# NVIDIA/nvidia-resiliency-ext

Hardware: AMD Instinct MI355X
Metric: generate_report_latency_us (lower is better)
Workload: dtype f32; 1 GPU; 8 ranks x 64 sections x 10000 samples per report, ring capacity 10000, relative+individual scores, gather_on_rank0; logical_ranks_per_gpu=8, rows_per_gpu=512, exchange=none (single process)

## Files before the change

nvidia-resiliency-ext_amd/csrc/nvrx_straggler.hip:

```cpp
#include <hip/hip_runtime.h>
#include <hip/hip_ext.h>

#include <algorithm>
#include <atomic>
#include <chrono>
#include <thread>
#include <cmath>
#include <cstdarg>
#include <cstdio>
#include <cstdlib>
#include <cstring>
#include <deque>
#include <mutex>
#include <string>
#include <unordered_map>
#include <utility>
#include <vector>

#include "nvrx_straggler.h"

namespace {

thread_local std::string g_err;

// ... 282 lines not shown
    mn = min(mn, dpp<DPP_QUAD_2301>(0xFFFFFFFFu, mn));
    mx = max(mx, dpp0<DPP_QUAD_2301>(mx));
    mn = min(mn, dpp<DPP_ROW_SHR4>(0xFFFFFFFFu, mn));
    mx = max(mx, dpp0<DPP_ROW_SHR4>(mx));
    mn = min(mn, dpp<DPP_ROW_SHR8>(0xFFFFFFFFu, mn));
    mx = max(mx, dpp0<DPP_ROW_SHR8>(mx));
    mn = min(mn, dpp<DPP_BCAST15>(0xFFFFFFFFu, mn));
    mx = max(mx, dpp0<DPP_BCAST15>(mx));
    mn = min(mn, dpp<DPP_BCAST31>(0xFFFFFFFFu, mn));
    mx = max(mx, dpp0<DPP_BCAST31>(mx));
    mn = (uint32_t)__builtin_amdgcn_readlane((int)mn, 63);
    mx = (uint32_t)__builtin_amdgcn_readlane((int)mx, 63);
}

__device__ __forceinline__ double recip_count(uint32_t c) {
    const double d = (double)c;
    double r = __builtin_amdgcn_rcp(d);
    r = fma(fma(-d, r, 1.0), r, r);
    r = fma(fma(-d, r, 1.0), r, r);
    return c ? r : __builtin_inf();
}

template <int THREADS, int VPT>
__global__ __launch_bounds__(THREADS) void k_row_stats(const float *__restrict__ samples,
                                                       const uint32_t *__restrict__ counts,
                                                       const uint8_t *__restrict__ kinds, int row_stride,
                                                       float *__restrict__ stats, Epilogue ep, int uniform_n) {
    constexpr int WAVES = THREADS / 64;
    constexpr int HIST_BITS = THREADS >= 512 ? NVRX_HIST_BITS_WIDE : 11;
    constexpr int HIST_BINS = 1 << HIST_BITS;
    constexpr int PER = HIST_BINS / THREADS;
    constexpr int G = THREADS / 64;
    constexpr int NKEY = VPT * 4;
    constexpr int CAND_MAX = 256;
    constexpr int CAND_ONE = 64;
    static_assert(HIST_BINS % THREADS == 0, "THREADS must divide the histogram size");
    static_assert(THREADS >= CAND_MAX, "candidate list is initialised one word per thread");

    __shared__ __attribute__((aligned(16))) uint32_t s_hist[HIST_BINS];
    __shared__ __attribute__((aligned(16))) uint32_t s_sum[THREADS];
    __shared__ __attribute__((aligned(16))) uint32_t s_cand[CAND_MAX];
    __shared__ __attribute__((aligned(16))) uint32_t s_lt[CAND_MAX];
    __shared__ __attribute__((aligned(16))) double s_d[2 * WAVES];
    __shared__ __attribute__((aligned(16))) uint32_t s_mm[4];
    __shared__ uint32_t s_cur[1];

    const int row = ep.rows_active ? (int)(blockIdx.x / ep.rows_active) * ep.rows_per_rank + (int)(blockIdx.x % ep.rows_active)
                                   : (int)blockIdx.x;
    const int tid = threadIdx.x;
    const int lane = tid & 63;
// ... 487 lines not shown
                                              r_min, r_max, r_med, r_avg, r_std, (float)n, weight, (float)path};
#pragma unroll
            for (int q = 0; q < ROW_GRANULES; q++)
                __hip_atomic_store(g8 + q, tag | (unsigned long long)__float_as_uint(vals[q]), __ATOMIC_RELAXED,
                                   __HIP_MEMORY_SCOPE_AGENT);
        } else if (ep.send) {
            const int lr = row / ep.rows_per_rank;
            float *s = ep.send + (size_t)lr * ep.L;
            const int g = row_gid;
            if (g >= 0 && g < ep.KS) {
                s[g] = n ? r_med : -1.0f;
                s[ep.KS + g] = n ? h : __builtin_nanf("");
                if (g < ep.K) s[2 * ep.KS + g] = weight;
            }
            if (row - lr * ep.rows_per_rank == 0) s[ep.L - 1] = ep.names_ok;
        }
    }
    NVRX_PHASE(8);
#ifdef NVRX_PHASE_CLOCKS
    if (threadIdx.x == 0 && blockIdx.x < 4096) g_phase[blockIdx.x][9] = wall_clock64();
#endif
}

struct StagedSample {
    uint32_t row_slot;
    float value;
};

__global__ void k_scatter(const uint32_t *__restrict__ h_counts, const StagedSample *__restrict__ h_entries,
                          int n_entries, float *__restrict__ samples, int row_stride,
                          uint32_t *__restrict__ d_counts, int rows, const uint8_t *__restrict__ h_kinds,
                          uint8_t *__restrict__ d_kinds, const int32_t *__restrict__ h_gid,
                          int32_t *__restrict__ d_gid, uint32_t *__restrict__ done_cnt, uint32_t *done_word,
                          uint32_t ticket) {
    const int i = blockIdx.x * blockDim.x + threadIdx.x;
    if (i < n_entries) {
        const StagedSample e = h_entries[i];
        samples[(size_t)(e.row_slot >> 16) * (size_t)row_stride + (e.row_slot & 0xFFFFu)] = e.value;
    }
    if (i < rows) {
        d_counts[i] = h_counts[i];
        if (h_kinds) {
            d_kinds[i] = h_kinds[i];
            d_gid[i] = h_gid[i];
        }
    }
// ... 350 lines not shown
    float *send;
    nvrx_f4 *stats_out;
    uint32_t *err;
    int n_blocks, rows_active, rows_per_rank, local_ranks;
    float names_ok;
    uint32_t epoch;
    unsigned long long timeout_ticks;
    int poll_naps;
};

__device__ __forceinline__ float wait_granule(const unsigned long long *p, const GatherArgs &g, unsigned long long t0) {
    uint32_t spins = 0;
    for (;;) {
        const unsigned long long x = __hip_atomic_load(p, __ATOMIC_RELAXED, __HIP_MEMORY_SCOPE_AGENT);
        if ((uint32_t)(x >> 32) == g.epoch) return __uint_as_float((uint32_t)x);
        __builtin_amdgcn_s_sleep(2);
        if ((++spins & 0xFFu) == 0u && wall_clock64() - t0 > g.timeout_ticks) {
            __hip_atomic_store(g.err, g.epoch, __ATOMIC_RELAXED, __HIP_MEMORY_SCOPE_SYSTEM);
            return __builtin_nanf("");
        }
    }
}

template <int NTHR>
__global__ __launch_bounds__(NTHR) void k_score1(ScoreArgs a, int fence, PeerArgs pa, GatherArgs ga) {
    extern __shared__ __attribute__((aligned(16))) unsigned char s_raw[];

    const int K = a.K, S = a.S, KS = K + S, R = a.R;
    const int L = NVRX_TABLE_LEN(K, S);
    const int W = NVRX_SCORE_LEN(S);
    const int nout = R * W;
    const int nout4 = (nout + 3) & ~3;
    float *s_min = reinterpret_cast<float *>(s_raw);
    float *s_out = s_min + ((KS + 3) & ~3);
    uint8_t *s_fl = reinterpret_cast<uint8_t *>(s_out + nout4);
    float *s_tab = a.tab_in_lds ? reinterpret_cast<float *>(s_fl + ((nout + 15) & ~15)) : nullptr;
    float *s_send = a.tab_in_lds ? s_tab + ((R * L + 3) & ~3) : nullptr;
    const int tid = threadIdx.x;
    const float NaN = __builtin_nanf("");
    const unsigned long long t_begin = wall_clock64();
#if NVRX_TOUCH_KERNARGS
    {
        constexpr int KARG_DWORDS = (int)((sizeof(ScoreArgs) + sizeof(int) + sizeof(PeerArgs) + sizeof(GatherArgs)) / 4);
        const uint32_t __attribute__((address_space(4))) *ka =
            (const uint32_t __attribute__((address_space(4))) *)__builtin_amdgcn_kernarg_segment_ptr();
        uint32_t touched = 0u;
#pragma unroll
        for (int d = 0; d < KARG_DWORDS; d += 16) touched ^= ka[d];
        asm volatile("" ::"s"(touched));
    }
#endif
    const int pair_r0 = tid / max(S, 1), pair_s0 = tid - pair_r0 * S;
    const int pair_dr = NTHR / max(S, 1), pair_ds = NTHR - pair_dr * S;
    const bool lds_only = ga.g && s_send;
    auto sync = [&]() {
        if (lds_only)
            asm volatile("s_waitcnt lgkmcnt(0)\n\ts_barrier" ::: "memory");
        else
            __syncthreads();
    };

    if (ga.g && s_send) {
        for (int j = tid; j < a.send_floats; j += NTHR) {
            const int col = j % L;
            s_send[j] = col < KS ? -1.0f : (col < 2 * KS ? NaN : 0.0f);
        }
        __syncthreads();
    }
    if (ga.g) {
        constexpr int CH = 8;
        const int total = ga.n_blocks * 3;
        for (int base = tid; base < total; base += NTHR * CH) {
            unsigned long long x[CH];
            int slot[CH];
// ... 28 lines not shown
                        __hip_atomic_store(ga.err, ga.epoch, __ATOMIC_RELAXED, __HIP_MEMORY_SCOPE_SYSTEM);
                        v = NaN;
                        got = true;
                    }
                    if (got) {
                        if (slot[c] >= 0) {
                            ga.send[slot[c]] = v;
                            if (s_send) s_send[slot[c]] = v;
                        }
                        pending &= ~(1u << c);
                    }
                }
                if (pending) {
                    for (int nap = 0; nap < ga.poll_naps; nap++) __builtin_amdgcn_s_sleep(1);
                    spins++;
                }
            }
        }
        for (int lr = tid; lr < ga.local_ranks; lr += NTHR) {
            ga.send[(size_t)lr * L + (L - 1)] = ga.names_ok;
            if (s_send) s_send[lr * L + (L - 1)] = ga.names_ok;
        }
        sync();
    }
    const unsigned long long t_rows = wall_clock64();
    if (pa.windows) {
        peer_exchange_block(pa, ga.g ? s_send : nullptr, s_tab);
        __syncthreads();
        if (s_tab) a.table = s_tab;
    } else if (ga.g && s_send) {
        a.table = s_send;
    }
    for (int i = tid; i < a.stats_n4; i += NTHR) {
        const float4 v = a.stats_src[i];
        store16_sys(a.stats_dst + i, nvrx_f4{v.x, v.y, v.z, v.w});
    }
    auto score_all = [&](const float *tab) {
        score_colmin(a, tab, tid, NTHR, s_min);
        if (a.meta && (tid >> 6) == NTHR / 64 - 1) score_meta(a, tab, tid & 63);
        if (tid < nout4 - nout) s_out[nout + tid] = 0.f;
        if (tid < ((nout + 15) & ~15) - nout) s_fl[nout + tid] = 0;
        sync();

        {
            int r = pair_r0, sct = pair_s0;
#pragma unroll 2
// ... 94 lines not shown
        __hip_atomic_store(&a.meta[6], (uint32_t)(t_rows - t_begin), __ATOMIC_RELAXED, __HIP_MEMORY_SCOPE_SYSTEM);
        __hip_atomic_store(&a.meta[7], (uint32_t)min(wall_clock64() - t_rows, 0xFFFFull) | ((uint32_t)min(t_staged - t_rows, 0xFFFFull) << 16),
                           __ATOMIC_RELAXED, __HIP_MEMORY_SCOPE_SYSTEM);
        __hip_atomic_store(&a.meta[4], a.seq, __ATOMIC_RELAXED, __HIP_MEMORY_SCOPE_SYSTEM);
    }
    if (ga.g && ga.stats_out) {
        for (int idx = tid; idx < ga.n_blocks * 2; idx += NTHR) {
            const int b = idx >> 1, half = idx & 1;
            const unsigned long long *p = ga.g + (size_t)b * ROW_GRANULES + 3 + 4 * half;
            nvrx_f4 v;
            v.x = wait_granule(p + 0, ga, t_begin);
            v.y = wait_granule(p + 1, ga, t_begin);
            v.z = wait_granule(p + 2, ga, t_begin);
            v.w = wait_granule(p + 3, ga, t_begin);
            const int lr = b / ga.rows_active;
            const int row = lr * ga.rows_per_rank + (b - lr * ga.rows_active);
            store16_sys(ga.stats_out + (size_t)row * 2 + half, v);
        }
        asm volatile("s_waitcnt vmcnt(0)" ::: "memory");
        __syncthreads();
        if (tid == 0 && publish) __hip_atomic_store(&a.meta[5], a.seq, __ATOMIC_RELAXED, __HIP_MEMORY_SCOPE_SYSTEM);
    }
}

using StatsKernel = void (*)(const float *, const uint32_t *, const uint8_t *, int, float *, Epilogue, int);

struct StatsVariant {
    int threads;
    int vpt;
    StatsKernel fn;
};

#define SV(T, V) \
    { T, V, k_row_stats<T, V> }
const StatsVariant kVariants[] = {
    SV(256, 1),  SV(256, 2),  SV(256, 3),  SV(256, 4),  SV(256, 5),   SV(256, 6),  SV(256, 8),  SV(256, 10),
    SV(256, 12), SV(256, 16), SV(512, 1),  SV(512, 2),  SV(512, 3),   SV(512, 4),  SV(512, 5),  SV(512, 6),
    SV(512, 8),  SV(512, 10), SV(512, 12), SV(512, 16), SV(1024, 1),  SV(1024, 2), SV(1024, 3), SV(1024, 4),
    SV(1024, 5), SV(1024, 6), SV(1024, 8), SV(1024, 10), SV(1024, 12), SV(1024, 16),
};
#undef SV

const StatsVariant *pick_variant(int row_stride) {
    int prefs[3] = {512, 1024, 256};
    if (row_stride <= 256 * 4 * 2) {
        prefs[0] = 256;
// ... 172 lines not shown
    int wall_khz = 100000;
    int resident_mode = 1;
    int poll_naps = 4;
    int rehome_mode = 1;
    bool side_work = true;
    uint64_t reports_rehomed = 0;
    int last_rehome_verdict = 0;
    uint64_t side_gen = 1, async_gen = 0;
    bool async_on_ctx = false;
    double last_report_us = 0.0;
    double async_rehome_gap_us = 5000.0;
    hipEvent_t report_ev = nullptr;
    uint64_t report_epoch = 0;
    hipStream_t guard_stream = nullptr;
    bool guard_recorded = true;
    bool stamps_used = false;
    uint64_t guard_done_epoch = 0;
    struct StreamEpoch {
        hipStream_t stream;
        uint64_t epoch;
    };
    std::vector<StreamEpoch> stream_epochs;

    std::mutex mu;
};

static bool stream_is_capturing(hipStream_t st);
static void stamp_slot_give(int slot);

namespace {

int ctx_set_device(const nvrx_ctx *ctx) {
    HIP_TRY(hipSetDevice(ctx->device));
    return NVRX_OK;
}

inline void mark_side_work(nvrx_ctx *ctx) {
    ctx->side_work = true;
    ctx->side_gen++;
}

int guard_ring_writer(nvrx_ctx *ctx, hipStream_t st) {
    if (!ctx->report_epoch) return NVRX_OK;
    nvrx_ctx::StreamEpoch *se = nullptr;
    for (auto &e : ctx->stream_epochs)
        if (e.stream == st) se = &e;
    if (!se) {
        ctx->stream_epochs.push_back({st, 0});
        se = &ctx->stream_epochs.back();
    }
    if (se->epoch < ctx->report_epoch) {
// ... 159 lines not shown
extern "C" {

int nvrx_abi_version(void) { return NVRX_ABI_VERSION; }

int nvrx_report_desc_size(void) { return (int)sizeof(nvrx_report_desc); }

const char *nvrx_last_error(void) { return g_err.c_str(); }

int nvrx_row_stats(const float *d_samples, const uint32_t *d_counts, const uint8_t *d_kinds, int rows,
                   int row_stride, float *d_stats, void *stream) {
    if (rows < 0 || row_stride <= 0 || (row_stride & 3)) return fail(NVRX_ERR_INVALID, "row_stride must be a positive multiple of 4 (got %d), rows >= 0", row_stride);
    if (rows > 0 && (!d_samples || !d_counts || !d_stats)) return fail(NVRX_ERR_INVALID, "null device pointer");
    if ((reinterpret_cast<uintptr_t>(d_samples) & 15u) != 0) return fail(NVRX_ERR_INVALID, "d_samples must be 16-byte aligned");
    Epilogue ep{};
    return launch_row_stats(d_samples, d_counts, d_kinds, rows, row_stride, d_stats, ep, as_stream(stream));
}

static bool score_fits_single_wg(int R, int K, int S, const float *d_scores, const uint8_t *d_flags) {
    return R <= SCORE1_MAX_RANKS && score1_lds_bytes(R, K, S) <= SCORE1_MAX_LDS &&
           (reinterpret_cast<uintptr_t>(d_scores) & 15u) == 0 && (reinterpret_cast<uintptr_t>(d_flags) & 15u) == 0 &&
           score_single_wg_enabled();
}

static int score_launch(const float *d_table, int R, int K, int S, int do_indiv, int do_rel, const double *thresholds,
                        float *d_scores, uint8_t *d_flags, uint32_t *d_meta, uint32_t *d_done_counter, uint32_t seq,
                        const float *d_stats_src, float *d_stats_dst, int stats_rows, void *stream, const PeerArgs *pa,
                        const GatherArgs *ga = nullptr) {
    if (R <= 0 || K < 0 || S < 0) return fail(NVRX_ERR_INVALID, "bad table shape R=%d K=%d S=%d", R, K, S);
    if (!d_table || !d_scores) return fail(NVRX_ERR_INVALID, "null device pointer");
    hipStream_t st = as_stream(stream);
    ScoreArgs a{};
    a.table = d_table;
    a.R = R;
    a.K = K;
    a.S = S;
    a.do_indiv = do_indiv;
    a.do_rel = do_rel;
    for (int i = 0; i < 4; i++) a.thr[i] = thresholds ? thresholds[i] : 0.75;
    a.scores = d_scores;
    a.flags = d_flags;
    a.meta = d_meta;
    a.done_counter = d_meta ? d_done_counter : nullptr;
    a.seq = seq;
    if (d_stats_src && d_stats_dst && stats_rows > 0) {
        a.stats_src = reinterpret_cast<const float4 *>(d_stats_src);
        a.stats_dst = reinterpret_cast<float4 *>(d_stats_dst);
        a.stats_n4 = stats_rows * (NVRX_STATS_STRIDE / 4);
    }
    const int KS = K + S;
    if (score_fits_single_wg(R, K, S, d_scores, d_flags)) {
        PeerArgs none{};
        GatherArgs nog{};
        size_t lds1 = score1_lds_bytes(R, K, S);
        if (ga || pa) {
            const int send_floats = pa ? pa->count : R * NVRX_TABLE_LEN(K, S);
            const size_t extra = score1_table_lds_bytes(R, K, S, send_floats);
            if (lds1 + extra <= SCORE1_MAX_LDS) {
                a.tab_in_lds = 1;
                a.send_floats = send_floats;
                lds1 += extra;
            }
        }
        if (ga) {
            a.stats_n4 = 0;
            hipLaunchKernelGGL(k_score1<SCORE1_RESIDENT_THREADS>, dim3(1), dim3(SCORE1_RESIDENT_THREADS), lds1, st, a,
                               score_fence_enabled(), pa ? *pa : none, *ga);
        } else {
            report_clk(7);
            hipLaunchKernelGGL(k_score1<SCORE1_THREADS>, dim3(1), dim3(SCORE1_THREADS), lds1, st, a, score_fence_enabled(),
                               pa ? *pa : none, nog);
        }
        HIP_TRY(hipGetLastError());
        return NVRX_OK;
    }
    if (ga) return fail(NVRX_ERR_STATE, "the resident scorer needs the single-workgroup score kernel");
    if (pa) return fail(NVRX_ERR_STATE, "the exchange prologue needs the single-workgroup score kernel");
    size_t lds = (size_t)KS * sizeof(float);
    int tile_ranks = 0;
    if (R > 64 || lds > 48 * 1024) {
        const int chunks = std::max(1, std::min(COLMIN_MAX_CHUNKS, (R + 63) / 64));
        const int rows_per_chunk = (R + chunks - 1) / chunks;
        const size_t need = (size_t)KS * (size_t)(chunks + 1);
        float *scratch = nullptr;
        {
            std::lock_guard<std::mutex> lk(g_scratch_mu);
// ... 58 lines not shown
    HIP_TRY(hipSetDevice(device));

    nvrx_ctx *ctx = new (std::nothrow) nvrx_ctx();
    if (!ctx) return fail(NVRX_ERR_NOMEM, "host allocation failed");
    ctx->device = device;
    ctx->local_ranks = local_ranks;
    ctx->rows_per_rank = rows_per_rank;
    ctx->rows = local_ranks * rows_per_rank;
    ctx->ring_cap = ring_cap;
    ctx->row_stride = (ring_cap + 3) & ~3;
    ctx->stage_cap = 4096;
    ctx->total.assign((size_t)ctx->rows, 0);
    ctx->stage_cnt.assign((size_t)ctx->rows, 0);
    ctx->stage_gen.assign((size_t)ctx->rows, 0);
    ctx->resident_mode = resident_scorer_mode_from_env();
    ctx->poll_naps = poll_naps_from_env();
    {
        const char *e = getenv("NVRX_DEBUG_REPORT_REHOME");
        ctx->rehome_mode = (e && atoi(e) == 0) ? 0 : 1;
        const char *g = getenv("NVRX_DEBUG_ASYNC_REHOME_GAP_US");
        if (g && *g) ctx->async_rehome_gap_us = atof(g);
        const char *eg = getenv("NVRX_DEBUG_EAGER_GUARD");
        ctx->stamps_used = eg && atoi(eg) != 0;
    }

#define CTX_TRY(expr)                                                                         \
    do {                                                                                      \
        hipError_t e_ = (expr);                                                               \
        if (e_ != hipSuccess) {                                                               \
            int rc_ = fail(NVRX_ERR_HIP, "%s failed: %s", #expr, hipGetErrorString(e_));      \
            nvrx_ctx_destroy(ctx);                                                            \
            return rc_;                                                                       \
        }                                                                                     \
    } while (0)

    const size_t nsamp = (size_t)ctx->rows * (size_t)ctx->row_stride;
    CTX_TRY(hipMalloc(reinterpret_cast<void **>(&ctx->d_samples), nsamp * sizeof(float)));
    CTX_TRY(hipMemset(ctx->d_samples, 0, nsamp * sizeof(float)));
    CTX_TRY(hipMalloc(reinterpret_cast<void **>(&ctx->d_counts), (size_t)ctx->rows * sizeof(uint32_t)));
    CTX_TRY(hipMemset(ctx->d_counts, 0, (size_t)ctx->rows * sizeof(uint32_t)));
    CTX_TRY(hipMalloc(reinterpret_cast<void **>(&ctx->d_kinds), (size_t)ctx->rows));
    CTX_TRY(hipMemset(ctx->d_kinds, 0, (size_t)ctx->rows));
    CTX_TRY(hipMalloc(reinterpret_cast<void **>(&ctx->d_gid), (size_t)ctx->rows * sizeof(int32_t)));
    CTX_TRY(hipMemset(ctx->d_gid, 0xFF, (size_t)ctx->rows * sizeof(int32_t)));
    CTX_TRY(hipMalloc(reinterpret_cast<void **>(&ctx->d_hist_min), (size_t)ctx->rows * sizeof(float)));
    hipLaunchKernelGGL(k_fill_f32, dim3((ctx->rows + 255) / 256), dim3(256), 0, nullptr, ctx->d_hist_min, (size_t)ctx->rows, INFINITY);
// ... 10 lines not shown
    CTX_TRY(hipMemset(ctx->d_stage_cnt, 0, (size_t)nvrx_ctx::NBUF * sizeof(uint32_t)));
    {
        int bi = 0;
        for (StageBuf &b : ctx->buf) {
            CTX_TRY(hipHostMalloc(reinterpret_cast<void **>(&b.h_counts), (size_t)ctx->rows * sizeof(uint32_t), hipHostMallocDefault));
            CTX_TRY(hipHostMalloc(reinterpret_cast<void **>(&b.h_entries), (size_t)ctx->stage_cap * sizeof(StagedSample), hipHostMallocDefault));
            b.h_done = ctx->h_stage_done + (size_t)bi * 16;
            b.d_done = ctx->d_stage_done + (size_t)bi * 16;
            b.d_cnt = ctx->d_stage_cnt + bi;
            bi++;
        }
    }
    CTX_TRY(hipEventCreateWithFlags(&ctx->copy_done, hipEventDisableTiming));
    CTX_TRY(hipEventCreateWithFlags(&ctx->stamp_ev, hipEventDisableTiming));
    CTX_TRY(hipEventCreateWithFlags(&ctx->order_ev, hipEventDisableTiming));
    CTX_TRY(hipEventCreateWithFlags(&ctx->report_ev, hipEventDisableTiming));
    {
        const size_t gbytes = 2ull * (size_t)ctx->rows * ROW_GRANULES * sizeof(unsigned long long);
        CTX_TRY(hipMalloc(reinterpret_cast<void **>(&ctx->d_rowg), gbytes));
        CTX_TRY(hipMemset(ctx->d_rowg, 0, gbytes));
        CTX_TRY(hipHostMalloc(reinterpret_cast<void **>(&ctx->h_gather_err), 64, hipHostMallocMapped));
        ctx->h_gather_err[0] = 0;
        CTX_TRY(hipHostGetDevicePointer(reinterpret_cast<void **>(&ctx->d_gather_err), ctx->h_gather_err, 0));
    }
    ctx->stamps_argfree = true;
    if (ctx->stamps_argfree) {
        CTX_TRY(hipGetSymbolAddress(reinterpret_cast<void **>(&ctx->d_stamps), HIP_SYMBOL(g_stamp_slots)));
    } else {
        CTX_TRY(hipMalloc(reinterpret_cast<void **>(&ctx->d_stamps), nvrx_ctx::NSTAMP * sizeof(unsigned long long)));
        CTX_TRY(hipMemset(ctx->d_stamps, 0, nvrx_ctx::NSTAMP * sizeof(unsigned long long)));
    }
    {
        int khz = 0;
        if (hipDeviceGetAttribute(&khz, hipDeviceAttributeWallClockRate, device) == hipSuccess && khz > 0) {
            ctx->us_per_tick = 1000.0f / (float)khz;
            ctx->wall_khz = khz;
        }
    }
    CTX_TRY(hipDeviceSynchronize());
#undef CTX_TRY
    *out = ctx;
    return NVRX_OK;
}

int nvrx_ctx_destroy(nvrx_ctx *ctx) {
    if (!ctx) return NVRX_OK;
// ... 22 lines not shown
        (void)hipEventDestroy(p.end);
    }
    if (ctx->copy_done) (void)hipEventDestroy(ctx->copy_done);
    if (ctx->stamp_ev) (void)hipEventDestroy(ctx->stamp_ev);
    if (ctx->order_ev) (void)hipEventDestroy(ctx->order_ev);
    if (ctx->report_ev) (void)hipEventDestroy(ctx->report_ev);
    {
        std::lock_guard<std::mutex> lk(g_scratch_mu);
        ctx->report_streams.push_back(ctx->score_stream);
        for (hipStream_t rs : ctx->report_streams) {
            auto it = g_scratch_by_stream.find(reinterpret_cast<void *>(rs));
            if (it == g_scratch_by_stream.end()) continue;
            if (it->second.ptr) (void)hipFree(it->second.ptr);
            g_scratch_by_stream.erase(it);
        }
    }
    if (ctx->score_stream) (void)hipStreamDestroy(ctx->score_stream);
    if (ctx->d_rowg) (void)hipFree(ctx->d_rowg);
    if (ctx->h_gather_err) (void)hipHostFree(ctx->h_gather_err);
    if (ctx->d_stamps && !ctx->stamps_argfree) (void)hipFree(ctx->d_stamps);
    if (ctx->d_stamps_own) (void)hipFree(ctx->d_stamps_own);
    for (const auto &o : ctx->open_stamps)
        if (!o.own) stamp_slot_give(o.slot);
    delete ctx;
    return NVRX_OK;
}

int nvrx_ctx_set_stream(nvrx_ctx *ctx, void *stream) {
    if (!ctx) return fail(NVRX_ERR_INVALID, "ctx is null");
    std::lock_guard<std::mutex> lk(ctx->mu);
    ctx->default_stream = as_stream(stream);
    return NVRX_OK;
}

int nvrx_ctx_info(const nvrx_ctx *ctx, int what) {
    if (!ctx) return fail(NVRX_ERR_INVALID, "ctx is null");
    switch (what) {
        case 0: return ctx->local_ranks;
        case 1: return ctx->rows_per_rank;
        case 2: return ctx->ring_cap;
        case 3: return ctx->row_stride;
        case 4: return ctx->device;
        case 5: return (int)ctx->reports_rehomed;
        case 6: return ctx->last_rehome_verdict;
        case 7: return (int)ctx->regions_skipped;
        case 8: {
            std::lock_guard<std::mutex> lk(const_cast<nvrx_ctx *>(ctx)->mu);
            return ctx->rows_used;
        }
        default: return fail(NVRX_ERR_INVALID, "unknown info selector %d", what);
    }
}

int nvrx_row_configure(nvrx_ctx *ctx, int row, int kind, int gid) {
    if (!ctx) return fail(NVRX_ERR_INVALID, "ctx is null");
    if (row < 0 || row >= ctx->rows) return fail(NVRX_ERR_INVALID, "row %d out of range [0,%d)", row, ctx->rows);
    if (kind != NVRX_KIND_SECTION && kind != NVRX_KIND_KERNEL) return fail(NVRX_ERR_INVALID, "bad kind %d", kind);
    std::lock_guard<std::mutex> lk(ctx->mu);
    if (ctx->h_kinds[row] != (uint8_t)kind || ctx->h_gid[row] != gid) {
        ctx->h_kinds[row] = (uint8_t)kind;
        ctx->h_gid[row] = gid;
        touch_row(ctx, row);
        ctx->meta_dirty = true;
    }
    return NVRX_OK;
}

int nvrx_row_alloc(nvrx_ctx *ctx, int kind) {
    if (!ctx) return fail(NVRX_ERR_INVALID, "ctx is null");
    if (kind != NVRX_KIND_SECTION && kind != NVRX_KIND_KERNEL) return fail(NVRX_ERR_INVALID, "bad kind %d", kind);
    std::lock_guard<std::mutex> lk(ctx->mu);
// ... 486 lines not shown
        touch_row(ctx, row);
        float *dst_cpu = nullptr;
        if (cpu_row >= 0) {
            dst_cpu = ctx->d_samples + (size_t)cpu_row * (size_t)ctx->row_stride + (size_t)(ctx->total[(size_t)cpu_row] % cap);
            ctx->total[(size_t)cpu_row]++;
            touch_row(ctx, cpu_row);
        }
        ctx->counts_dirty = true;
        hipStream_t st = as_stream(stream);
        {
            int grc = guard_ring_writer(ctx, st);
            if (grc) return grc;
        }
        ctx->stamps_used = true;
        hipLaunchKernelGGL(k_stamp_end, dim3(1), dim3(1), 0, st, slot_ptr, ctx->us_per_tick, dst_gpu, dst_cpu, cpu_value);
        HIP_TRY(hipGetLastError());
        if (std::find(ctx->stamp_streams.begin(), ctx->stamp_streams.end(), st) == ctx->stamp_streams.end())
            ctx->stamp_streams.push_back(st);
        return NVRX_OK;
    }
    return fail(NVRX_ERR_STATE, "nvrx_stamp_end(row=%d) without a matching nvrx_stamp_begin", row);
}

static int report_local_impl(nvrx_ctx *ctx, float *d_stats, float *d_send, int K, int S, int names_ok, int rows_active,
                             void *stream, unsigned long long *rowg, uint32_t epoch);

int nvrx_report_local(nvrx_ctx *ctx, float *d_stats, float *d_send, int K, int S, int names_ok, int rows_active,
                      void *stream) {
    if (ctx) {
        std::lock_guard<std::mutex> lk(ctx->mu);
        mark_side_work(ctx);
    }
    return report_local_impl(ctx, d_stats, d_send, K, S, names_ok, rows_active, stream, nullptr, 0);
}

static int report_local_impl(nvrx_ctx *ctx, float *d_stats, float *d_send, int K, int S, int names_ok, int rows_active,
                             void *stream, unsigned long long *rowg, uint32_t epoch) {
    hipStream_t st = as_stream(stream);
    if (!ctx || !d_stats) return fail(NVRX_ERR_INVALID, "null argument");
    if (K < 0 || S < 0) return fail(NVRX_ERR_INVALID, "bad K/S");
    if (rows_active < 0 || rows_active > ctx->rows_per_rank) return fail(NVRX_ERR_INVALID, "rows_active %d outside [0,%d]", rows_active, ctx->rows_per_rank);
    if (rows_active == 0) rows_active = ctx->rows_per_rank;
    std::lock_guard<std::mutex> lk(ctx->mu);
    int rc = ctx_set_device(ctx);
    if (rc) return rc;
    int uniform_n = -1;
    rc = flush_locked(ctx, st, &uniform_n, rows_active);
    if (rc) return rc;
    report_clk(2);
    Epilogue ep{};
    ep.gid = ctx->d_gid;
    ep.hist_min = d_send ? ctx->d_hist_min : nullptr;
    ep.send = d_send;
    ep.rows_per_rank = ctx->rows_per_rank;
    ep.rows_active = rows_active;
    ep.K = K;
    ep.KS = K + S;
    ep.L = NVRX_TABLE_LEN(K, S);
    ep.names_ok = names_ok ? 1.0f : 0.0f;
    ep.rowg = rowg;
    ep.epoch = epoch;
    int pair = -1;
    hipEvent_t ev_start = nullptr, ev_stop = nullptr;
    if (ctx->timing) {
        rc = get_pair(ctx->timing_pairs, ctx->timing_free, &pair);
        if (rc) return rc;
        ev_start = ctx->timing_pairs[(size_t)pair].start;
        ev_stop = ctx->timing_pairs[(size_t)pair].end;
    }
    rc = launch_row_stats(ctx->d_samples, ctx->d_counts, ctx->d_kinds, ctx->local_ranks * rows_active, ctx->row_stride,
                          d_stats, ep, st, ev_start, ev_stop, uniform_n);
    if (rc) return rc;
    if (pair >= 0) ctx->timing_used.push_back(pair);
    report_clk(3);
    return NVRX_OK;
}

struct nvrx_peer {
    int device = 0, world = 0, rank = 0, stride = 0;
    unsigned long long *window = nullptr;
    std::vector<unsigned long long *> mapped;
    std::vector<bool> opened;
    unsigned long long **d_windows = nullptr;
    uint32_t *h_err = nullptr, *d_err = nullptr;
// ... 104 lines not shown
                    for (const char *var : {"WORLD_SIZE", "SLURM_NTASKS", "OMPI_COMM_WORLD_SIZE", "PMI_SIZE"}) {
                        const char *v = getenv(var);
                        if (!v || !*v) continue;
                        const long n = strtol(v, nullptr, 10);
                        if (n > 1) high = false;
                        if (n > 1 || strcmp(var, "WORLD_SIZE") == 0) break;
                    }
                }
                if (high) {
                    int least = 0, greatest = 0;
                    HIP_TRY(hipDeviceGetStreamPriorityRange(&least, &greatest));
                    HIP_TRY(hipStreamCreateWithPriority(&ctx->score_stream, hipStreamNonBlocking, greatest));
                } else {
                    HIP_TRY(hipStreamCreateWithFlags(&ctx->score_stream, hipStreamNonBlocking));
                }
            }
            if (d->order_after_enabled && d->order_after_stream != stream)
                HIP_TRY(hipStreamWaitEvent(ctx->score_stream, ctx->order_ev, 0));
            if (!ctx->stamp_streams.empty()) {
                int orc = order_after_stamps(ctx, as_stream(stream), ctx->score_stream);
                if (orc) return orc;
            }
        }
        ctx->gran_epoch = (ctx->gran_epoch % 0x7FFFFFFFu) + 1u;
        unsigned long long *slice = ctx->d_rowg + (size_t)(ctx->gran_epoch & 1u) * (size_t)ctx->rows * ROW_GRANULES;
        int rc2 = report_local_impl(ctx, d->d_stats, d->d_send, d->K, d->S, d->names_ok, d->rows_active, stream, slice,
                                    ctx->gran_epoch);
        if (rc2) return rc2;
        GatherArgs ga{};
        ga.g = slice;
        ga.gid = ctx->d_gid;
        ga.send = d->d_send;
        ga.stats_out = (d->d_stats_dst && d->stats_rows > 0) ? reinterpret_cast<nvrx_f4 *>(d->d_stats_dst) : nullptr;
        ga.err = ctx->d_gather_err;
        ga.n_blocks = rows_launch;
        ga.rows_active = d->rows_active > 0 ? d->rows_active : ctx->rows_per_rank;
        ga.rows_per_rank = ctx->rows_per_rank;
        ga.local_ranks = ctx->local_ranks;
        ga.names_ok = d->names_ok ? 1.0f : 0.0f;
        ga.epoch = ctx->gran_epoch;
        ga.timeout_ticks = (unsigned long long)((d->timeout_s > 0.0 ? d->timeout_s : 1e9) * 1e3 * (double)ctx->wall_khz);
        ga.poll_naps = ctx->poll_naps;
        PeerArgs pa{};
        if (peer_route) {
            rc2 = peer_fill_args(static_cast<nvrx_peer *>(d->comm), d->d_send, d->d_table, (size_t)d->send_count, &pa);
            if (rc2) return rc2;
        }
        d->seq = (d->seq % 0x7FFFFFFFu) + 1u;
        rc2 = score_launch(exchanging ? d->d_table : d->d_send, d->R, d->K, d->S, d->do_indiv, d->do_rel, d->thresholds,
                           d->d_scores, d->d_flags, d->d_meta, d->d_done_counter, d->seq, nullptr, nullptr, 0,
                           ctx->score_stream, peer_route ? &pa : nullptr, &ga);
        if (rc2) return rc2;
        report_clk(4);
        report_clk(5);
        rc2 = nvrx_poll_u32(d->h_seq_word, d->seq, d->timeout_s > 0.0 ? d->timeout_s : 1e30);
        report_clk(6);
        if (rc2) return rc2;
        if (*static_cast<volatile uint32_t *>(ctx->h_gather_err) == ctx->gran_epoch)
            return fail(NVRX_ERR_TIMEOUT, "the score kernel gave up waiting for the statistics kernel's rows (epoch %u)", ctx->gran_epoch);
        if (as_stream(stream) == ctx->default_stream) {
            std::lock_guard<std::mutex> lk(ctx->mu);
            ctx->side_work = false;
            ctx->async_on_ctx = false;
        }
        return NVRX_OK;
    }
    int rc = report_local_impl(ctx, d->d_stats, d->d_send, d->K, d->S, d->names_ok, d->rows_active, stream, nullptr, 0);
    if (rc) return rc;
    if (d->guard_rings) {
        std::lock_guard<std::mutex> lk(ctx->mu);
        ctx->guard_stream = as_stream(stream);
        if (rehomed || !ctx->stamps_used) {
            ctx->guard_recorded = false;
        } else {
            HIP_TRY(hipEventRecord(ctx->report_ev, as_stream(stream)));
            ctx->guard_recorded = true;
        }
        ctx->report_epoch++;
    }
    PeerArgs pa{};
    bool prologue = false;
    if (exchanging && d->allgather_fn == reinterpret_cast<void *>(&nvrx_peer_allgather) &&
// ... 357 lines not shown
```

Baseline: 27.77 us.

## Launch report kernels argument-free from constant-memory plans with device-side counters

Adds argument-free variants of the row-stats and single-workgroup score kernels. They read their parameters from a cached plan in __constant__ memory and take the epoch and sequence counters from a device word, which the score kernel advances itself. The host writes a plan only after the same plan has been seen twice in a row, and it synchronizes around that write. Steady-state reports can then launch with no kernel arguments, which is meant to cut launch and kernarg overhead. The cost is host-side plan bookkeeping, a global slot pool, and stream synchronizations whenever a plan or counter changes.

```diff
diff --git a/nvidia-resiliency-ext_amd/csrc/nvrx_straggler.hip b/nvidia-resiliency-ext_amd/csrc/nvrx_straggler.hip
--- a/nvidia-resiliency-ext_amd/csrc/nvrx_straggler.hip
+++ b/nvidia-resiliency-ext_amd/csrc/nvrx_straggler.hip
@@ -328,10 +328,9 @@
 }
 
 template <int THREADS, int VPT>
-__global__ __launch_bounds__(THREADS) void k_row_stats(const float *__restrict__ samples,
-                                                       const uint32_t *__restrict__ counts,
-                                                       const uint8_t *__restrict__ kinds, int row_stride,
-                                                       float *__restrict__ stats, Epilogue ep, int uniform_n) {
+__device__ __forceinline__ void row_stats_body(const float *__restrict__ samples, const uint32_t *__restrict__ counts,
+                                               const uint8_t *__restrict__ kinds, int row_stride,
+                                               float *__restrict__ stats, const Epilogue &ep, int uniform_n) {
     constexpr int WAVES = THREADS / 64;
     constexpr int HIST_BITS = THREADS >= 512 ? NVRX_HIST_BITS_WIDE : 11;
     constexpr int HIST_BINS = 1 << HIST_BITS;
@@ -865,6 +864,14 @@
 #endif
 }
 
+template <int THREADS, int VPT>
+__global__ __launch_bounds__(THREADS) void k_row_stats(const float *__restrict__ samples,
+                                                       const uint32_t *__restrict__ counts,
+                                                       const uint8_t *__restrict__ kinds, int row_stride,
+                                                       float *__restrict__ stats, Epilogue ep, int uniform_n) {
+    row_stats_body<THREADS, VPT>(samples, counts, kinds, row_stride, stats, ep, uniform_n);
+}
+
 struct StagedSample {
     uint32_t row_slot;
     float value;
@@ -1261,8 +1268,11 @@
     }
 }
 
+__host__ __device__ constexpr uint32_t report_counter_next(uint32_t v) { return (v % 0x7FFFFFFFu) + 1u; }
+
 template <int NTHR>
-__global__ __launch_bounds__(NTHR) void k_score1(ScoreArgs a, int fence, PeerArgs pa, GatherArgs ga) {
+__device__ __forceinline__ void score1_body(ScoreArgs a, int fence, PeerArgs pa, GatherArgs ga, uint32_t *adv_epoch,
+                                            uint32_t *adv_seq) {
     extern __shared__ __attribute__((aligned(16))) unsigned char s_raw[];
 
     const int K = a.K, S = a.S, KS = K + S, R = a.R;
@@ -1278,17 +1288,6 @@
     const int tid = threadIdx.x;
     const float NaN = __builtin_nanf("");
     const unsigned long long t_begin = wall_clock64();
-#if NVRX_TOUCH_KERNARGS
-    {
-        constexpr int KARG_DWORDS = (int)((sizeof(ScoreArgs) + sizeof(int) + sizeof(PeerArgs) + sizeof(GatherArgs)) / 4);
-        const uint32_t __attribute__((address_space(4))) *ka =
-            (const uint32_t __attribute__((address_space(4))) *)__builtin_amdgcn_kernarg_segment_ptr();
-        uint32_t touched = 0u;
-#pragma unroll
-        for (int d = 0; d < KARG_DWORDS; d += 16) touched ^= ka[d];
-        asm volatile("" ::"s"(touched));
-    }
-#endif
     const int pair_r0 = tid / max(S, 1), pair_s0 = tid - pair_r0 * S;
     const int pair_dr = NTHR / max(S, 1), pair_ds = NTHR - pair_dr * S;
     const bool lds_only = ga.g && s_send;
@@ -1363,6 +1362,10 @@
             if (s_send) s_send[lr * L + (L - 1)] = ga.names_ok;
         }
         sync();
+        if (adv_epoch && tid == 0) {
+            __hip_atomic_store(adv_epoch, report_counter_next(ga.epoch), __ATOMIC_RELAXED, __HIP_MEMORY_SCOPE_AGENT);
+            __hip_atomic_store(adv_seq, report_counter_next(a.seq), __ATOMIC_RELAXED, __HIP_MEMORY_SCOPE_AGENT);
+        }
     }
     const unsigned long long t_rows = wall_clock64();
     if (pa.windows) {
@@ -1503,6 +1506,86 @@
         if (tid == 0 && publish) __hip_atomic_store(&a.meta[5], a.seq, __ATOMIC_RELAXED, __HIP_MEMORY_SCOPE_SYSTEM);
     }
 }
+
+template <int NTHR>
+__global__ __launch_bounds__(NTHR) void k_score1(ScoreArgs a, int fence, PeerArgs pa, GatherArgs ga) {
+#if NVRX_TOUCH_KERNARGS
+    {
+        constexpr int KARG_DWORDS = (int)((sizeof(ScoreArgs) + sizeof(int) + sizeof(PeerArgs) + sizeof(GatherArgs)) / 4);
+        const uint32_t __attribute__((address_space(4))) *ka =
+            (const uint32_t __attribute__((address_space(4))) *)__builtin_amdgcn_kernarg_segment_ptr();
+        uint32_t touched = 0u;
+#pragma unroll
+        for (int d = 0; d < KARG_DWORDS; d += 16) touched ^= ka[d];
+        asm volatile("" ::"s"(touched));
+    }
+#endif
+    score1_body<NTHR>(a, fence, pa, ga, nullptr, nullptr);
+}
+
+constexpr int NVRX_NPLAN = 16;
+constexpr int NVRX_NPLAN_PER_CTX = 4;
+constexpr int PLAN_ROW_THREADS = 512;
+struct ReportPlan {
+    const float *samples;
+    const uint32_t *counts;
+    const uint8_t *kinds;
+    int row_stride;
+    float *stats;
+    Epilogue ep;
+    int uniform_n;
+    ScoreArgs sa;
+    int fence;
+    GatherArgs ga;
+    size_t rowg_half;
+    uint32_t *ctr;
+};
+__constant__ ReportPlan g_plans[NVRX_NPLAN];
+
+template <int SLOT, int VPT>
+__global__ __launch_bounds__(PLAN_ROW_THREADS) void k_row_stats_at() {
+    const ReportPlan &p = g_plans[SLOT];
+    Epilogue ep = p.ep;
+    ep.epoch = __hip_atomic_load(p.ctr, __ATOMIC_RELAXED, __HIP_MEMORY_SCOPE_AGENT);
+    ep.rowg = p.ep.rowg + (size_t)(ep.epoch & 1u) * p.rowg_half;
+    row_stats_body<PLAN_ROW_THREADS, VPT>(p.samples, p.counts, p.kinds, p.row_stride, p.stats, ep, p.uniform_n);
+}
+
+template <int SLOT>
+__global__ __launch_bounds__(SCORE1_RESIDENT_THREADS) void k_score1_at() {
+    const ReportPlan &p = g_plans[SLOT];
+#if NVRX_TOUCH_KERNARGS
+    {
+        const uint32_t __attribute__((address_space(4))) *ka = (const uint32_t __attribute__((address_space(4))) *)&p;
+        uint32_t touched = 0u;
+#pragma unroll
+        for (int d = 0; d < (int)(sizeof(ReportPlan) / 4); d += 16) touched ^= ka[d];
+        asm volatile("" ::"s"(touched));
+    }
+#endif
+    GatherArgs ga = p.ga;
+    ScoreArgs a = p.sa;
+    ga.epoch = __hip_atomic_load(p.ctr, __ATOMIC_RELAXED, __HIP_MEMORY_SCOPE_AGENT);
+    a.seq = __hip_atomic_load(p.ctr + 1, __ATOMIC_RELAXED, __HIP_MEMORY_SCOPE_AGENT);
+    ga.g += (size_t)(ga.epoch & 1u) * p.rowg_half;
+    __syncthreads();
+    score1_body<SCORE1_RESIDENT_THREADS>(a, p.fence, PeerArgs{}, ga, p.ctr, p.ctr + 1);
+}
+
+using PlanKernel = void (*)();
+template <int VPT, int... I>
+static const PlanKernel *plan_row_table(std::integer_sequence<int, I...>) {
+    static const PlanKernel table[] = {k_row_stats_at<I, VPT>...};
+    return table;
+}
+template <int... I>
+static const PlanKernel *plan_score_table(std::integer_sequence<int, I...>) {
+    static const PlanKernel table[] = {k_score1_at<I>...};
+    return table;
+}
+static const PlanKernel *const g_plan_row_fn[2] = {plan_row_table<4>(std::make_integer_sequence<int, NVRX_NPLAN>{}),
+                                                   plan_row_table<5>(std::make_integer_sequence<int, NVRX_NPLAN>{})};
+static const PlanKernel *const g_plan_score_fn = plan_score_table(std::make_integer_sequence<int, NVRX_NPLAN>{});
 
 using StatsKernel = void (*)(const float *, const uint32_t *, const uint8_t *, int, float *, Epilogue, int);
 
@@ -1721,11 +1804,47 @@
     };
     std::vector<StreamEpoch> stream_epochs;
 
+    struct PlanSlot {
+        const void *desc;
+        int slot;
+        bool written;
+        ReportPlan dev;
+        bool cand_valid;
+        ReportPlan cand;
+        uint64_t last_use;
+    };
+    int argfree_mode = 1;
+    std::vector<PlanSlot> plans;
+    uint32_t *d_plan_ctr = nullptr;
+    uint32_t plan_ctr[2] = {0, 0};
+    bool plan_ctr_synced = false;
+    uint64_t plan_uses = 0;
+    uint64_t reports_argfree = 0, plan_writes = 0;
+
     std::mutex mu;
 };
 
 static bool stream_is_capturing(hipStream_t st);
 static void stamp_slot_give(int slot);
+
+static std::mutex g_plan_slot_mu;
+static uint32_t g_plan_slot_held = 0;
+static_assert(NVRX_NPLAN <= 32, "the held-slot mask is one 32-bit word");
+
+static int plan_slot_take() {
+    std::lock_guard<std::mutex> lk(g_plan_slot_mu);
+    for (int i = 0; i < NVRX_NPLAN; i++)
+        if (!(g_plan_slot_held >> i & 1u)) {
+            g_plan_slot_held |= 1u << i;
+            return i;
+        }
+    return -2;
+}
+
+static void plan_slot_give(int slot) {
+    std::lock_guard<std::mutex> lk(g_plan_slot_mu);
+    g_plan_slot_held &= ~(1u << slot);
+}
 
 namespace {
 
@@ -1931,13 +2050,9 @@
            score_single_wg_enabled();
 }
 
-static int score_launch(const float *d_table, int R, int K, int S, int do_indiv, int do_rel, const double *thresholds,
-                        float *d_scores, uint8_t *d_flags, uint32_t *d_meta, uint32_t *d_done_counter, uint32_t seq,
-                        const float *d_stats_src, float *d_stats_dst, int stats_rows, void *stream, const PeerArgs *pa,
-                        const GatherArgs *ga = nullptr) {
-    if (R <= 0 || K < 0 || S < 0) return fail(NVRX_ERR_INVALID, "bad table shape R=%d K=%d S=%d", R, K, S);
-    if (!d_table || !d_scores) return fail(NVRX_ERR_INVALID, "null device pointer");
-    hipStream_t st = as_stream(stream);
+static ScoreArgs make_score_args(const float *d_table, int R, int K, int S, int do_indiv, int do_rel, const double *thresholds,
+                                 float *d_scores, uint8_t *d_flags, uint32_t *d_meta, uint32_t *d_done_counter, uint32_t seq,
+                                 const float *d_stats_src, float *d_stats_dst, int stats_rows) {
     ScoreArgs a{};
     a.table = d_table;
     a.R = R;
@@ -1956,20 +2071,37 @@
         a.stats_dst = reinterpret_cast<float4 *>(d_stats_dst);
         a.stats_n4 = stats_rows * (NVRX_STATS_STRIDE / 4);
     }
+    return a;
+}
+
+static size_t score1_launch_lds(ScoreArgs &a, bool prologue, const PeerArgs *pa) {
+    size_t lds1 = score1_lds_bytes(a.R, a.K, a.S);
+    if (prologue) {
+        const int send_floats = pa ? pa->count : a.R * NVRX_TABLE_LEN(a.K, a.S);
+        const size_t extra = score1_table_lds_bytes(a.R, a.K, a.S, send_floats);
+        if (lds1 + extra <= SCORE1_MAX_LDS) {
+            a.tab_in_lds = 1;
+            a.send_floats = send_floats;
+            lds1 += extra;
+        }
+    }
+    return lds1;
+}
+
+static int score_launch(const float *d_table, int R, int K, int S, int do_indiv, int do_rel, const double *thresholds,
+                        float *d_scores, uint8_t *d_flags, uint32_t *d_meta, uint32_t *d_done_counter, uint32_t seq,
+                        const float *d_stats_src, float *d_stats_dst, int stats_rows, void *stream, const PeerArgs *pa,
+                        const GatherArgs *ga = nullptr) {
+    if (R <= 0 || K < 0 || S < 0) return fail(NVRX_ERR_INVALID, "bad table shape R=%d K=%d S=%d", R, K, S);
+    if (!d_table || !d_scores) return fail(NVRX_ERR_INVALID, "null device pointer");
+    hipStream_t st = as_stream(stream);
+    ScoreArgs a = make_score_args(d_table, R, K, S, do_indiv, do_rel, thresholds, d_scores, d_flags, d_meta, d_done_counter,
+                                  seq, d_stats_src, d_stats_dst, stats_rows);
     const int KS = K + S;
     if (score_fits_single_wg(R, K, S, d_scores, d_flags)) {
         PeerArgs none{};
         GatherArgs nog{};
-        size_t lds1 = score1_lds_bytes(R, K, S);
-        if (ga || pa) {
-            const int send_floats = pa ? pa->count : R * NVRX_TABLE_LEN(K, S);
-            const size_t extra = score1_table_lds_bytes(R, K, S, send_floats);
-            if (lds1 + extra <= SCORE1_MAX_LDS) {
-                a.tab_in_lds = 1;
-                a.send_floats = send_floats;
-                lds1 += extra;
-            }
-        }
+        const size_t lds1 = score1_launch_lds(a, ga || pa, pa);
         if (ga) {
             a.stats_n4 = 0;
             hipLaunchKernelGGL(k_score1<SCORE1_RESIDENT_THREADS>, dim3(1), dim3(SCORE1_RESIDENT_THREADS), lds1, st, a,
@@ -2074,6 +2206,8 @@
         if (g && *g) ctx->async_rehome_gap_us = atof(g);
         const char *eg = getenv("NVRX_DEBUG_EAGER_GUARD");
         ctx->stamps_used = eg && atoi(eg) != 0;
+        const char *ea = getenv("NVRX_DEBUG_ARGFREE_REPORT");
+        ctx->argfree_mode = (ea && atoi(ea) == 0) ? 0 : 1;
     }
 
 #define CTX_TRY(expr)                                                                         \
@@ -2130,6 +2264,7 @@
         CTX_TRY(hipHostMalloc(reinterpret_cast<void **>(&ctx->h_gather_err), 64, hipHostMallocMapped));
         ctx->h_gather_err[0] = 0;
         CTX_TRY(hipHostGetDevicePointer(reinterpret_cast<void **>(&ctx->d_gather_err), ctx->h_gather_err, 0));
+        CTX_TRY(hipMalloc(reinterpret_cast<void **>(&ctx->d_plan_ctr), 64));
     }
     ctx->stamps_argfree = true;
     if (ctx->stamps_argfree) {
@@ -2198,6 +2333,8 @@
     if (ctx->d_stamps_own) (void)hipFree(ctx->d_stamps_own);
     for (const auto &o : ctx->open_stamps)
         if (!o.own) stamp_slot_give(o.slot);
+    for (const auto &ps : ctx->plans) plan_slot_give(ps.slot);
+    if (ctx->d_plan_ctr) (void)hipFree(ctx->d_plan_ctr);
     delete ctx;
     return NVRX_OK;
 }
@@ -2223,6 +2360,14 @@
         case 8: {
             std::lock_guard<std::mutex> lk(const_cast<nvrx_ctx *>(ctx)->mu);
             return ctx->rows_used;
+        }
+        case 9: {
+            std::lock_guard<std::mutex> lk(const_cast<nvrx_ctx *>(ctx)->mu);
+            return (int)ctx->reports_argfree;
+        }
+        case 10: {
+            std::lock_guard<std::mutex> lk(const_cast<nvrx_ctx *>(ctx)->mu);
+            return (int)ctx->plan_writes;
         }
         default: return fail(NVRX_ERR_INVALID, "unknown info selector %d", what);
     }
@@ -2755,8 +2900,19 @@
     return fail(NVRX_ERR_STATE, "nvrx_stamp_end(row=%d) without a matching nvrx_stamp_begin", row);
 }
 
+struct ArgfreeScore {
+    const void *desc;
+    ScoreArgs sa;
+    size_t lds;
+    int fence;
+    GatherArgs ga;
+    uint32_t seq;
+    bool used;
+    int slot;
+};
+
 static int report_local_impl(nvrx_ctx *ctx, float *d_stats, float *d_send, int K, int S, int names_ok, int rows_active,
-                             void *stream, unsigned long long *rowg, uint32_t epoch);
+                             void *stream, unsigned long long *rowg, uint32_t epoch, ArgfreeScore *af = nullptr);
 
 int nvrx_report_local(nvrx_ctx *ctx, float *d_stats, float *d_send, int K, int S, int names_ok, int rows_active,
                       void *stream) {
@@ -2767,8 +2923,87 @@
     return report_local_impl(ctx, d_stats, d_send, K, S, names_ok, rows_active, stream, nullptr, 0);
 }
 
+static int report_plan_launch(nvrx_ctx *ctx, hipStream_t st, float *d_stats, const Epilogue &ep, int uniform_n, int rows,
+                              uint32_t epoch, ArgfreeScore *af) {
+    af->used = false;
+    const StatsVariant *v = pick_variant(ctx->row_stride);
+    if (!ctx->argfree_mode || ctx->timing || rows <= 0 || !v || v->threads != PLAN_ROW_THREADS || (v->vpt != 4 && v->vpt != 5))
+        return NVRX_OK;
+    nvrx_ctx::PlanSlot *ps = nullptr;
+    for (auto &q : ctx->plans)
+        if (q.desc == af->desc) ps = &q;
+    if (!ps) {
+        if ((int)ctx->plans.size() >= NVRX_NPLAN_PER_CTX) {
+            ps = &ctx->plans[0];
+            for (auto &q : ctx->plans)
+                if (q.last_use < ps->last_use) ps = &q;
+            const int slot = ps->slot;
+            *ps = nvrx_ctx::PlanSlot{};
+            ps->slot = slot;
+        } else {
+            const int slot = plan_slot_take();
+            if (slot < 0) return NVRX_OK;
+            ctx->plans.push_back(nvrx_ctx::PlanSlot{});
+            ps = &ctx->plans.back();
+            ps->slot = slot;
+        }
+        ps->desc = af->desc;
+    }
+    ps->last_use = ++ctx->plan_uses;
+    ReportPlan p;
+    memset(&p, 0, sizeof p);
+    p.samples = ctx->d_samples;
+    p.counts = ctx->d_counts;
+    p.kinds = ctx->d_kinds;
+    p.row_stride = ctx->row_stride;
+    p.stats = d_stats;
+    p.ep = ep;
+    p.ep.rowg = ctx->d_rowg;
+    p.ep.epoch = 0;
+    p.uniform_n = uniform_n;
+    p.sa = af->sa;
+    p.sa.seq = 0;
+    p.fence = af->fence;
+    p.ga = af->ga;
+    p.ga.g = ctx->d_rowg;
+    p.ga.epoch = 0;
+    p.rowg_half = (size_t)ctx->rows * ROW_GRANULES;
+    p.ctr = ctx->d_plan_ctr;
+    const uint32_t ctr[2] = {epoch, af->seq};
+    const bool same = ps->written && memcmp(&p, &ps->dev, sizeof p) == 0;
+    if (!same || !ctx->plan_ctr_synced || ctx->plan_ctr[0] != ctr[0] || ctx->plan_ctr[1] != ctr[1]) {
+        if (!same && !(ps->cand_valid && memcmp(&p, &ps->cand, sizeof p) == 0)) {
+            ps->cand = p;
+            ps->cand_valid = true;
+            return NVRX_OK;
+        }
+        ps->written = false;
+        ctx->plan_ctr_synced = false;
+        HIP_TRY(hipStreamSynchronize(st));
+        HIP_TRY(hipStreamSynchronize(ctx->score_stream));
+        if (!same)
+            HIP_TRY(hipMemcpyToSymbolAsync(HIP_SYMBOL(g_plans), &p, sizeof p, (size_t)ps->slot * sizeof(ReportPlan),
+                                           hipMemcpyHostToDevice, st));
+        HIP_TRY(hipMemcpyAsync(ctx->d_plan_ctr, ctr, sizeof ctr, hipMemcpyHostToDevice, st));
+        HIP_TRY(hipStreamSynchronize(st));
+        ps->dev = p;
+        ps->written = true;
+        ps->cand_valid = false;
+        ctx->plan_writes++;
+    }
+    hipLaunchKernelGGL(g_plan_row_fn[v->vpt - 4][ps->slot], dim3(rows), dim3(PLAN_ROW_THREADS), 0, st);
+    HIP_TRY(hipGetLastError());
+    ctx->plan_ctr[0] = report_counter_next(epoch);
+    ctx->plan_ctr[1] = report_counter_next(af->seq);
+    ctx->plan_ctr_synced = true;
+    ctx->reports_argfree++;
+    af->slot = ps->slot;
+    af->used = true;
+    return NVRX_OK;
+}
+
 static int report_local_impl(nvrx_ctx *ctx, float *d_stats, float *d_send, int K, int S, int names_ok, int rows_active,
-                             void *stream, unsigned long long *rowg, uint32_t epoch) {
+                             void *stream, unsigned long long *rowg, uint32_t epoch, ArgfreeScore *af) {
     hipStream_t st = as_stream(stream);
     if (!ctx || !d_stats) return fail(NVRX_ERR_INVALID, "null argument");
     if (K < 0 || S < 0) return fail(NVRX_ERR_INVALID, "bad K/S");
@@ -2793,6 +3028,14 @@
     ep.names_ok = names_ok ? 1.0f : 0.0f;
     ep.rowg = rowg;
     ep.epoch = epoch;
+    if (af) {
+        rc = report_plan_launch(ctx, st, d_stats, ep, uniform_n, ctx->local_ranks * rows_active, epoch, af);
+        if (rc) return rc;
+        if (af->used) {
+            report_clk(3);
+            return NVRX_OK;
+        }
+    }
     int pair = -1;
     hipEvent_t ev_start = nullptr, ev_stop = nullptr;
     if (ctx->timing) {
@@ -2943,11 +3186,8 @@
                 if (orc) return orc;
             }
         }
-        ctx->gran_epoch = (ctx->gran_epoch % 0x7FFFFFFFu) + 1u;
+        ctx->gran_epoch = report_counter_next(ctx->gran_epoch);
         unsigned long long *slice = ctx->d_rowg + (size_t)(ctx->gran_epoch & 1u) * (size_t)ctx->rows * ROW_GRANULES;
-        int rc2 = report_local_impl(ctx, d->d_stats, d->d_send, d->K, d->S, d->names_ok, d->rows_active, stream, slice,
-                                    ctx->gran_epoch);
-        if (rc2) return rc2;
         GatherArgs ga{};
         ga.g = slice;
         ga.gid = ctx->d_gid;
@@ -2962,23 +3202,50 @@
         ga.epoch = ctx->gran_epoch;
         ga.timeout_ticks = (unsigned long long)((d->timeout_s > 0.0 ? d->timeout_s : 1e9) * 1e3 * (double)ctx->wall_khz);
         ga.poll_naps = ctx->poll_naps;
+        const uint32_t seq = report_counter_next(d->seq);
+        ArgfreeScore af{};
+        if (!peer_route) {
+            af.desc = d;
+            af.sa = make_score_args(d->d_send, d->R, d->K, d->S, d->do_indiv, d->do_rel, d->thresholds, d->d_scores,
+                                    d->d_flags, d->d_meta, d->d_done_counter, seq, nullptr, nullptr, 0);
+            af.lds = score1_launch_lds(af.sa, true, nullptr);
+            af.fence = score_fence_enabled();
+            af.ga = ga;
+            af.seq = seq;
+        }
+        int rc2 = report_local_impl(ctx, d->d_stats, d->d_send, d->K, d->S, d->names_ok, d->rows_active, stream, slice,
+                                    ctx->gran_epoch, peer_route ? nullptr : &af);
+        if (rc2) return rc2;
+        auto drop_plan = [&](int rc) {
+            if (rc && af.used) {
+                std::lock_guard<std::mutex> lk(ctx->mu);
+                ctx->plan_ctr_synced = false;
+            }
+            return rc;
+        };
         PeerArgs pa{};
         if (peer_route) {
             rc2 = peer_fill_args(static_cast<nvrx_peer *>(d->comm), d->d_send, d->d_table, (size_t)d->send_count, &pa);
             if (rc2) return rc2;
         }
-        d->seq = (d->seq % 0x7FFFFFFFu) + 1u;
-        rc2 = score_launch(exchanging ? d->d_table : d->d_send, d->R, d->K, d->S, d->do_indiv, d->do_rel, d->thresholds,
-                           d->d_scores, d->d_flags, d->d_meta, d->d_done_counter, d->seq, nullptr, nullptr, 0,
-                           ctx->score_stream, peer_route ? &pa : nullptr, &ga);
-        if (rc2) return rc2;
+        d->seq = seq;
+        if (af.used) {
+            hipLaunchKernelGGL(g_plan_score_fn[af.slot], dim3(1), dim3(SCORE1_RESIDENT_THREADS), af.lds, ctx->score_stream);
+            const hipError_t le = hipGetLastError();
+            rc2 = le == hipSuccess ? NVRX_OK : fail(NVRX_ERR_HIP, "argument-free score launch failed: %s", hipGetErrorString(le));
+        } else {
+            rc2 = score_launch(exchanging ? d->d_table : d->d_send, d->R, d->K, d->S, d->do_indiv, d->do_rel, d->thresholds,
+                               d->d_scores, d->d_flags, d->d_meta, d->d_done_counter, d->seq, nullptr, nullptr, 0,
+                               ctx->score_stream, peer_route ? &pa : nullptr, &ga);
+        }
+        if (rc2) return drop_plan(rc2);
         report_clk(4);
         report_clk(5);
         rc2 = nvrx_poll_u32(d->h_seq_word, d->seq, d->timeout_s > 0.0 ? d->timeout_s : 1e30);
         report_clk(6);
-        if (rc2) return rc2;
+        if (rc2) return drop_plan(rc2);
         if (*static_cast<volatile uint32_t *>(ctx->h_gather_err) == ctx->gran_epoch)
-            return fail(NVRX_ERR_TIMEOUT, "the score kernel gave up waiting for the statistics kernel's rows (epoch %u)", ctx->gran_epoch);
+            return drop_plan(fail(NVRX_ERR_TIMEOUT, "the score kernel gave up waiting for the statistics kernel's rows (epoch %u)", ctx->gran_epoch));
         if (as_stream(stream) == ctx->default_stream) {
             std::lock_guard<std::mutex> lk(ctx->mu);
             ctx->side_work = false;
```

Result: faster. 26.85 us (median of 6 runs) (-3.3%).
